# JVBSouza/descriptools

Hardware: AMD Instinct MI355X
Metric: Mcells/s full descriptor chain (higher is better)
Workload: dtype f32; 1 GPU; 16384x16384 synthetic tilted-integer-fBm DEM per GPU, full chain (d8, flowacc, river mask, flowhand/HAND with fused GFI + ln(hl/H), fused slope+TI+MTI, downslope), device-resident; global_dem=16384x16384, river_threshold_cells=524288

## Files before the change

descriptools_amd/csrc/dt_capi.hip:

```cpp
#include <cmath>
#include <stdarg.h>
#include <stdlib.h>

#include <sys/mman.h>
#include <atomic>
#include <chrono>
#include <mutex>
#include <system_error>
#include <thread>
#include <utility>
#include <vector>

#include "dt_common.h"
#include "dt_kernels.h"

static thread_local char g_err[512] = "";
void dt_set_error(const char *fmt, ...) {
  va_list ap;
  va_start(ap, fmt);
  vsnprintf(g_err, sizeof(g_err), fmt, ap);
  va_end(ap);
}
extern "C" const char *dt_last_error(void) { return g_err; }
extern "C" const char *dt_version(void) { return "descriptools_hip 0.1 (gfx950)"; }
// ... 1135 lines not shown
}

static int dev_flowacc_river_flowhand_local(dt_ctx *c, const uint8_t *fdr, const float *dem, const uint8_t *nod4,
                                           int64_t H, int64_t W, int64_t threshold, int32_t *acc32, int8_t *river,
                                           const DtTwiEpilogue *twi = nullptr) {
  DT_CTX(c);
  DT_TRY(dt_check_hw(H, W));
  DT_REQUIRE((fdr && acc32 && river) || H * W == 0, "NULL raster");
  DT_REQUIRE(!twi || H * W == 0 || dt_twi_epilogue_ok(dt_full_window(H, W), acc32, river, twi),
             "this raster does not take the TI / MTI epilogue (dt_slope_from_d8_ok): use dt_dev_slope_twi");
  size_t need = dt_flowacc_tiled_scratch(H, W), need2 = dt_flowhand_tiled_scratch(H, W);
  DT_TRY(dt_scratch_reset(c, need + need2 + 512));
  void *scr = dt_scratch_take(c, need), *scr2 = dt_scratch_take(c, need2);
  DT_REQUIRE(scr && scr2, "scratch reservation failed");
  DtWin w = dt_full_window(H, W);
  DT_TRY(dt_launch_fa_local(c->stream, w, fdr, scr, need, acc32, 0));
  DT_TRY(dt_launch_fa_finish_fh_local(c->stream, w, fdr, dem, scr, scr2, need2, nullptr, threshold, acc32, 0, river,
                                      c->status, nod4, dt_nodata4_ld(W), twi));
  DT_HIP(hipGetLastError());
  c->scratch_owner = 2;
  c->owner_h = H;
  c->owner_w = W;
  c->owner_ptr = (char *)scr2;
  c->owner_ptr2 = nullptr;
  return DT_OK;
}
extern "C" int dt_dev_flowacc_river_flowhand_local(dt_ctx *c, const uint8_t *fdr, const float *dem, int64_t H, int64_t W,
                                                   int64_t threshold, int32_t *acc32, int8_t *river) {
  return dev_flowacc_river_flowhand_local(c, fdr, dem, nullptr, H, W, threshold, acc32, river);
}
extern "C" int dt_dev_flowacc_river_flowhand_local_m(dt_ctx *c, const uint8_t *fdr, const float *dem,
                                                     const uint8_t *nodata4, int64_t H, int64_t W, int64_t threshold,
                                                     int32_t *acc32, int8_t *river) {
// ... 1117 lines not shown
```

descriptools_amd/csrc/dt_common.h:

```cpp
#pragma once
#include <hip/hip_runtime.h>
#include <stdint.h>
#include <stdio.h>
#include <string.h>

#include "../../include/descriptools_hip.h"

#define DT_NODATA (-100.0f)

void dt_set_error(const char *fmt, ...);

#define DT_HIP(call)                                                                   \
  do {                                                                                 \
    hipError_t e__ = (call);                                                           \
    if (e__ != hipSuccess) {                                                           \
      dt_set_error("%s failed: %s (%s:%d)", #call, hipGetErrorString(e__), __FILE__,   \
                   __LINE__);                                                          \
      return e__ == hipErrorOutOfMemory ? DT_ENOMEM : DT_EHIP;                         \
    }                                                                                  \
  } while (0)

#define DT_REQUIRE(cond, msg)                      \
  do {                                             \
    if (!(cond)) {                                 \
      dt_set_error("invalid argument: %s", msg);   \
      return DT_EINVAL;                            \
    }                                              \
  } while (0)

#define DT_TRY(expr)          \
  do {                        \
    int rc__ = (expr);        \
    if (rc__ != DT_OK) return rc__; \
  } while (0)

enum { DT_DBG_TWI_FLAG_ALL = 0, DT_DBG_TWI_PLAIN = 1, DT_DBG_TWI_WX = 2, DT_DBG_TWI_MAP = 3, DT_DBG_DS_MARGIN = 4, DT_DBG_NO_FUSED_FA_FH = 5, DT_DBG_HY_FILL_SWEEPS = 6, DT_DBG_HY_FLAT_SWEEPS = 7, DT_DBG_HY_COLOUR_MIN = 8 , DT_DBG_FA_SCATTER = 9 , DT_DBG_RC_SLOTS = 10 , DT_DBG_COUNT = 11 };
#define DT_TWI_WX_DEFAULT 1
int dt_debug_get(int key);

struct dt_ctx {
  int device;
  hipStream_t stream;
  bool own_stream;
  char *scratch;
  size_t scratch_bytes;
  size_t scratch_used;
  int scratch_owner;
  int64_t owner_h, owner_w;
  char *owner_ptr;
  char *owner_ptr2;
  char *scratch2;
// ... 36 lines not shown
__host__ __device__ __forceinline__ bool dt_readable(const DtWin &w, int y, int x) {
  int gy = w.gy0 + y, gx = w.gx0 + x;
  return gy >= 0 && gy < w.Hg && gx >= 0 && gx < w.Wg && y >= -w.halo && y < w.H + w.halo && x >= -w.halo &&
         x < w.W + w.halo;
}
__host__ __device__ __forceinline__ bool dt_has_code(const DtWin &w, int y, int x) {
  if (!dt_readable(w, y, x)) return false;
  const int gy = w.gy0 + y, gx = w.gx0 + x;
  return (y > -w.halo || gy == 0) && (y < w.H + w.halo - 1 || gy == w.Hg - 1) && (x > -w.halo || gx == 0) &&
         (x < w.W + w.halo - 1 || gx == w.Wg - 1);
}
__host__ __device__ __forceinline__ bool dt_in_global(const DtWin &w, int y, int x) {
  int gy = w.gy0 + y, gx = w.gx0 + x;
  return gy >= 0 && gy < w.Hg && gx >= 0 && gx < w.Wg;
}
__host__ __device__ __forceinline__ long long dt_perim_count(int H, int W) {
  if (H <= 0 || W <= 0) return 0;
  if (H == 1) return W;
  if (W == 1) return H;
  return 2ll * W + 2ll * (H - 2);
}
__host__ __device__ __forceinline__ long long dt_perim_index(int H, int W, int y, int x) {
  if (H == 1) return x;
  if (W == 1) return y;
  if (y == 0) return x;
  if (y == H - 1) return (long long)W + x;
  if (x == 0) return 2ll * W + (y - 1);
  if (x == W - 1) return 2ll * W + (H - 2) + (y - 1);
  return -1;
}
// ... 9 lines not shown
```

descriptools_amd/csrc/dt_fa3fh1_kernel.inc:

```
#if FA3_TWI
__global__ __launch_bounds__(256, 6) void k_fa3fh1_twi(const uint8_t *__restrict__ fdr, const float *__restrict__ dem,
#else
template <int ND>
__global__ __launch_bounds__(256, 6) void k_fa3fh1(const uint8_t *__restrict__ fdr, const float *__restrict__ dem,
#endif
                                                  const uint8_t *__restrict__ nod4, int ldm, DtWin w, int tiles_x,
                                                  const unsigned long long *__restrict__ rec,
                                                  const unsigned long long *__restrict__ state,
                                                  const unsigned long long *__restrict__ ext,
                                                  const uint16_t *__restrict__ loc16, int32_t *__restrict__ acc32,
                                                  int32_t river_thr, int8_t *__restrict__ river,
                                                  int *__restrict__ status, uint32_t nnodes,
                                                  unsigned long long *__restrict__ nodes,
                                                  unsigned long long *__restrict__ cache,
#if FA3_TWI
                                                  uint8_t *__restrict__ cache_wide, TwiOut tw) {
  constexpr int ND = 2;
#else
                                                  uint8_t *__restrict__ cache_wide) {
#endif
#define P3(c) ((uint32_t)(c) + (((uint32_t)(c) >> 6) << 2))
#define NT3 (TH * (TW + 4))
  __shared__ __attribute__((aligned(16))) unsigned char smem[NT3 * 6];
  __shared__ unsigned long long s_in;
  __shared__ int s_ovf;
  uint32_t *s_delta = reinterpret_cast<uint32_t *>(smem);
  uint16_t *s_nxt = reinterpret_cast<uint16_t *>(smem + NT3 * 4);
  const int tile = dt_tile_of_block((int)blockIdx.x, (int)gridDim.x);
  const int ty = tile / tiles_x, tx = tile - ty * tiles_x;
  const int y0 = ty * TH, x0 = tx * TW;
  const uint4 v_fdr = dt_tile_fetch16(fdr, w, y0, x0);
  uint32_t c2[8] = {0u, 0u, 0u, 0u, 0u, 0u, 0u, 0u};
  if (rec) fa_nbr_codes(fdr, w, y0, x0, threadIdx.x, c2);
  unsigned long long e = 0ull;
// ... 29 lines not shown
    const bool interior = dt_tile_interior(w, y0, x0);
    const int pbase = ly * (TW + 4) + lxb;
#pragma unroll
    for (int q = 0; q < 4; q++) {
      uint32_t nn[4];
#pragma unroll
      for (int k = 0; k < 4; k++) {
        const uint32_t code = (cv[q] >> (8 * k)) & 0xFFu;
        const int lx = lxb + 4 * q + k;
        const uint32_t n = interior ? dt_tile_next_interior(code, ly, lx) : dt_tile_next(code, ly, lx, y0, x0, w);
        nn[k] = n < NT ? P3(n) : n;
      }
      *reinterpret_cast<uint2 *>(&s_nxt[pbase + 4 * q]) = make_uint2(nn[0] | (nn[1] << 16), nn[2] | (nn[3] << 16));
      *reinterpret_cast<uint4 *>(&s_delta[pbase + 4 * q]) = make_uint4(0, 0, 0, 0);
    }
  }
  if (rec) e = fa_inflow(fa_gather(c2, y0, x0, threadIdx.x, tiles_x, rec, state), e);
  if (threadIdx.x == 0) s_ovf = 0;
  if (__syncthreads_or(!(e & FA_CYCLE) && FA_VALUE(e) >= (1ull << 22))) {
    if (threadIdx.x == 0) s_in = 0ull;
    __syncthreads();
    if (e != 0ull && !(e & FA_CYCLE)) atomicAdd(&s_in, FA_VALUE(e));
    __syncthreads();
    if (threadIdx.x == 0 && s_in >= (1ull << 31) - (unsigned long long)NT && status) atomicOr(status, DT_STATUS_ACC_OVERFLOW);
  }
  if (e != 0ull) {
    int ly, lx;
    dt_cell_of_slot(threadIdx.x, ly, lx);
    uint32_t c = P3(ly * TW + lx);
    if (e & FA_CYCLE) {
// ... 57 lines not shown
        tw.tile_mark[stile] = (uint8_t)1;
      }
    }
#endif
  }
  __syncthreads();
#undef P3
#undef NT3
  uint32_t *s_w = reinterpret_cast<uint32_t *>(smem);
  uint8_t *s_fdr = smem + NT * 4;
  uint8_t *s_kind = smem + NT * 5;
  uint32_t *s_lut = reinterpret_cast<uint32_t *>(smem + NT * 6);
  s_lut[threadIdx.x] = fh_lut_entry(threadIdx.x);
  dt_tile_put16(s_fdr, v_fdr);
  __syncthreads();
  fh_tile1n_body(s_fdr, s_w, s_kind, &s_ovf, s_lut, riv4, w, tile, tiles_x, y0, x0, nnodes, nodes, cache, cache_wide);
}
```

descriptools_amd/csrc/dt_kernels.h:

```cpp
#pragma once
#include "dt_common.h"

int dt_launch_synth_dem(hipStream_t s, uint32_t seed, int O, int64_t Hg, int64_t y0, int64_t x0,
                        int64_t h, int64_t w, int nodata_pct, float *out);
int dt_launch_stencil(hipStream_t s, const DtWin &w, const float *dem, double px, float *slope,
                      uint8_t *fdr, float *slope_rad, const void *acc, int acc64, double n_top, float *ti,
                      float *mti, void *aux = nullptr, uint8_t *nod4 = nullptr, int ldm = 0);
static inline int dt_nodata4_ld(int64_t W) { return (int)((((W + 3) / 4) + 7) & ~(int64_t)7); }
static inline size_t dt_nodata4_bytes(int64_t H, int64_t W) { return (size_t)((H + 3) / 4) * (size_t)dt_nodata4_ld(W) * 2; }
size_t dt_stencil_aux_bytes(int64_t H, int64_t W);
int dt_launch_d8_slope(hipStream_t s, const DtWin &w, const float *dem, double px, uint8_t *fdr, float *slope,
                       void *aux, uint8_t *nod4, int ldm, void *smarks);
int dt_launch_slope_twi_fix(hipStream_t s, const DtWin &w, const float *dem, double px, float *slope,
                            const int32_t *acc, double n_top, float *ti, float *mti, void *smarks);
int dt_launch_flowacc(hipStream_t s, const uint8_t *fdr, const float *dem, int64_t H, int64_t W,
                      unsigned long long *state, int32_t *acc32);
int dt_launch_river_mask(hipStream_t s, const int32_t *acc32, int64_t n, int64_t thr, int8_t *river);
int dt_launch_flowhand(hipStream_t s, const float *dem, const uint8_t *fdr, const int8_t *river,
                       const int32_t *acc32, int64_t H, int64_t W, double px,
                       unsigned long long *state, float *fdist, int32_t *idx32, float *hand,
                       int32_t *a_river);
int dt_launch_twi(hipStream_t s, const int32_t *acc32, const float *srad, int64_t n, double px,
                  double n_top, float *ti, float *mti);
int dt_launch_twi_i64(hipStream_t s, const int64_t *fac, const float *srad, int64_t n, double px,
// ... 48 lines not shown
                             const int64_t *idx64, const void *fac, const void *a_river, int acc64, int64_t n_remote,
                             const uint8_t *res_ok, const int64_t *rem_gidx, const double *rem_zr64, void *table,
                             double expo, double b, double size, double *hand, float *gfi, float *lnhlh);
int dt_launch_ds_walk_f64(hipStream_t s, const DtWin &w, const double *dem, const uint8_t *fdr, double px, double dz,
                          int64_t n, void *rec, float *out);
int dt_launch_ds_walk_seed_f64(hipStream_t s, const DtWin &w, const double *dem, int64_t n, const int32_t *ys,
                               const int32_t *xs, void *rec);
int dt_launch_confusion(hipStream_t s, const double *desc, const int8_t *flood, int64_t n,
                        double nodata, const double *th_host, int nth, int under,
                        unsigned long long *counts4);
int dt_launch_i32_to_i64(hipStream_t s, const int32_t *a, int64_t n, int64_t *b);
int dt_launch_i64_to_i32(hipStream_t s, const int64_t *a, int64_t n, int32_t *b);

size_t dt_flowacc_tiled_scratch(int64_t H, int64_t W);
int dt_launch_fa_local(hipStream_t s, const DtWin &w, const uint8_t *fdr, void *scratch, size_t scratch_bytes,
                       int32_t *acc32, int rank_level);
int dt_launch_fa_summary(hipStream_t s, const DtWin &w, void *scratch, int64_t *A, int32_t *xr, uint8_t *code);
int dt_launch_fa_finish(hipStream_t s, const DtWin &w, const uint8_t *fdr, const float *dem, void *scratch,
                        const unsigned long long *ext_perim, int64_t river_thr, void *acc, int acc64,
                        int8_t *river, int *status = nullptr);
size_t dt_flowacc_weighted_scratch(int64_t H, int64_t W);
int dt_launch_flowacc_weighted(hipStream_t s, const DtWin &w, const uint8_t *fdr, const float *dem, const double *wt,
                               int frac_bits, void *scratch, size_t scratch_bytes, double *acc, int *status);
size_t dt_flowhand_tiled_scratch(int64_t H, int64_t W);
struct DtTwiEpilogue {
  const float *slope;
  float *ti, *mti;
  double px, n_top;
  void *marks;
};
int dt_launch_fa_finish_fh_local(hipStream_t s, const DtWin &w, const uint8_t *fdr, const float *dem, void *fa_scratch,
                                 void *fh_scratch, size_t fh_bytes, const unsigned long long *ext_perim,
                                 int64_t river_thr, void *acc, int acc64, int8_t *river, int *status,
                                 const uint8_t *nod4 = nullptr, int ldm = 0, const DtTwiEpilogue *twi = nullptr);
bool dt_twi_epilogue_ok(const DtWin &w, const void *acc, const int8_t *river, const DtTwiEpilogue *twi);
int dt_launch_fh_local(hipStream_t s, const DtWin &w, const uint8_t *fdr, const int8_t *river, void *scratch,
                       size_t scratch_bytes);
int dt_launch_fh_summary(hipStream_t s, const DtWin &w, void *scratch, const float *dem, const void *acc, int acc64,
                         uint8_t *kind, int32_t *ref, int32_t *nc, int32_t *nd, float *zr, long long *ar);
int dt_launch_fh_finish(hipStream_t s, const DtWin &w, const float *dem, const uint8_t *fdr,
                        const int8_t *river, const void *acc, int acc64, double px, void *scratch,
                        const uint8_t *res_ok, const int32_t *res_nc, const int32_t *res_nd,
                        const long long *rem_gidx, const float *rem_zr, const long long *rem_ar, float *fdist,
                        int32_t *idx32, long long *idx64, float *hand, void *a_river, float *gfi = nullptr,
                        float *lnhlh = nullptr, double n_gfi = 0.0, double b_gfi = 1.0, double size = 1.0);
int dt_launch_gfi_both(hipStream_t s, const float *hand, const void *a_river, const void *fac, int acc64,
                       int64_t n, double expo, double b, double size, float *gfi, float *lnhlh);
int dt_launch_unique_extremes(hipStream_t s, const float *x, int64_t n, uint32_t *work4, float *out3);
int dt_launch_minmax_scale(hipStream_t s, const float *x, int64_t n, float mn, float mx, float nodata,
// ... 69 lines not shown
```

descriptools_amd/csrc/dt_tiles.hip:

```cpp
#include "dt_common.h"
#include "dt_kernels.h"
#include "dt_math.h"

#define TW 64
#define TH 64
#define NT (TW * TH)
#define PS (2 * TW + 2 * (TH - 2))
#define CPT (NT / 256)

#define NX_SINK 0xFFFFu
#define NX_EXIT 0xFFFEu
#define NX_REXIT 0xFFFDu
#define X_NONE 0xFFFFu

__device__ __forceinline__ int dt_slot_of(int ly, int lx) {
  if (ly == 0) return lx;
  if (ly == TH - 1) return TW + lx;
  if (lx == 0) return 2 * TW + (ly - 1);
  if (lx == TW - 1) return 2 * TW + (TH - 2) + (ly - 1);
  return -1;
}
__device__ __forceinline__ void dt_cell_of_slot(int s, int &ly, int &lx) {
  if (s < TW) { ly = 0; lx = s; }
  else if (s < 2 * TW) { ly = TH - 1; lx = s - TW; }
// ... 270 lines not shown
  }
#pragma unroll
  for (int j = 0; j < CPT / 2; j++) {
    int c2 = threadIdx.x + 256 * j;
    uint32_t cy = *reinterpret_cast<const uint16_t *>(&s_cyc[2 * c2]);
    uint32_t a = (cy & 0xFFu) ? 0xFFFFu : (va[j] - 1u) & 0xFFFFu;
    uint32_t b = (cy & 0xFF00u) ? 0xFFFFu : (vb[j] - 1u) & 0xFFFFu;
    *reinterpret_cast<uint32_t *>(loc16 + (size_t)tile * NT + 2 * c2) = a | (b << 16);
  }
}

__global__ __launch_bounds__(256) void k_fa_reduce(const unsigned long long *__restrict__ rec, int64_t nnodes,
                                                  const uint32_t *__restrict__ entry_of,
                                                  const uint32_t *__restrict__ parent,
                                                  unsigned long long *__restrict__ state,
                                                  unsigned long long *__restrict__ ext) {
  const int64_t n = (int64_t)blockIdx.x * 256 + threadIdx.x;
  if (ext) {
    if (n >= nnodes) return;
    unsigned long long r = rec[n];
    if (REC_CODE(r) == 0) return;
    if (state[n] != 0ull) return;
    unsigned long long A = REC_W(r);
    uint32_t e = entry_of[n], p = parent[n];
    for (int64_t it = 0; it < nnodes; it++) {
      if (e == FA_NONE) break;
      atomicAdd(&ext[e], A);
      if (p == FA_NONE) break;
      unsigned long long rp = rec[p];
      uint32_t ep = entry_of[p], pp = parent[p];
      unsigned long long old = atomicAdd(&state[p], A - (1ull << FA2_SH));
      if ((old >> FA2_SH) != 1ull) break;
// ... 354 lines not shown
  return f;
}
struct FaIn {
  const unsigned long long *rec, *state, *ext;
};
static FaIn fa_inputs(const FaScratch &f, const unsigned long long *ext_perim) {
  if (dt_debug_get(DT_DBG_FA_SCATTER)) return FaIn{nullptr, nullptr, f.ext};
  return FaIn{f.rec, f.state, ext_perim ? f.ext : nullptr};
}
size_t dt_flowacc_tiled_scratch(int64_t H, int64_t W) {
  int64_t ntiles = ((W + TW - 1) / TW) * ((H + TH - 1) / TH);
  size_t nn = (size_t)ntiles * PS;
  return dt_align256(nn * 8) * 3 + dt_align256(nn * 4) * 3 + 256 + dt_align256((size_t)ntiles * NT * 2);
}

int dt_launch_fa_local(hipStream_t s, const DtWin &w, const uint8_t *fdr, void *scratch, size_t scratch_bytes,
                       int32_t *acc32, int rank_level) {
  if (w.H == 0 || w.W == 0) return DT_OK;
  DT_REQUIRE(scratch_bytes >= dt_flowacc_tiled_scratch(w.H, w.W), "scratch too small");
  FaScratch f = fa_layout(w, scratch);
  DT_REQUIRE(f.nnodes < 0x7FFFFFF0ll, "raster too large for one device tile");
  dim3 gt((unsigned)f.ntiles), b(256), gn((unsigned)((f.nnodes + 255) / 256));
  (void)acc32;
  const bool scatter = dt_debug_get(DT_DBG_FA_SCATTER) != 0;
  hipLaunchKernelGGL(k_fa_tile1, gt, b, 0, s, fdr, w, f.tiles_x, f.rec, f.loc16, f.state,
                     (rank_level || scatter) ? f.ext : nullptr, f.entry_of, f.parent);
  hipLaunchKernelGGL(k_fa_reduce, gn, b, 0, s, f.rec, f.nnodes, f.entry_of, f.parent, f.state, scatter ? f.ext : nullptr);
  if (rank_level) {
    hipLaunchKernelGGL(k_fa_nxt_init, gn, b, 0, s, f.rec, f.nnodes, f.entry_of, f.state, f.nxt);
  }
  return DT_OK;
}

int dt_launch_fa_summary(hipStream_t s, const DtWin &w, void *scratch, int64_t *A, int32_t *xr,
                         uint8_t *code) {
  int64_t P = dt_perim_count(w.H, w.W);
  if (P == 0) return DT_OK;
  FaScratch f = fa_layout(w, scratch);
  hipLaunchKernelGGL(k_fa_rank_summary, dim3((unsigned)((P + 255) / 256)), dim3(256), 0, s, w, f.tiles_x,
                     f.rec, f.state, f.nxt, f.nnodes, P, A, xr, code);
  return DT_OK;
}
// ... 498 lines not shown
  return (ptr & 0x7FFFu) | ((uint32_t)((s >> 16) & 0xFFu) << 15) | ((uint32_t)(s & 0xFFu) << 23);
}
__device__ __forceinline__ unsigned long long fh_cache_unpack(uint32_t v) {
  return fht_pack(v & 0x7FFFu, (v >> 15) & 0xFFu, ((v >> 23) & 0xFFu) | FHT_DONE);
}
__device__ __forceinline__ unsigned long long fh_cache_get(const unsigned long long *__restrict__ cache, bool wide,
                                                            int tile, int c) {
  if (wide) return cache[(size_t)tile * NT + c];
  return fh_cache_unpack(reinterpret_cast<const uint32_t *>(cache + (size_t)tile * NT)[c]);
}

__global__ __launch_bounds__(256) void k_fh_tile1(const uint8_t *__restrict__ fdr,
                                                 const int8_t *__restrict__ river, DtWin w, int tiles_x,
                                                 uint32_t nnodes, unsigned long long *__restrict__ nodes,
                                                 unsigned long long *__restrict__ cache,
                                                 uint8_t *__restrict__ cache_wide, int only_marked, int ntiles) {
  __shared__ __attribute__((aligned(16))) uint8_t s_fdr[NT];
  __shared__ uint8_t s_halo[2 * (TW + 2) + 2 * TH];
  __shared__ __attribute__((aligned(16))) unsigned long long s_st[NT];
  for (int tile = (int)blockIdx.x; tile < ntiles; tile += (int)gridDim.x) {
  if (only_marked && cache_wide[tile] != 2) continue;
  const int ty = tile / tiles_x, tx = tile - ty * tiles_x;
  const int y0 = ty * TH, x0 = tx * TW;
  FhTile T{s_fdr, s_halo, s_st};
  fht_solve_tile(T, fdr, river, w, y0, x0);
  if (threadIdx.x < PS) {
    int ly, lx;
    dt_cell_of_slot(threadIdx.x, ly, lx);
    unsigned long long s = s_st[ly * TW + lx];
    uint32_t ptr = (uint32_t)(s >> 32), nd = (uint32_t)((s >> 16) & 0xFFFFu);
    uint32_t ncf = (uint32_t)(s & 0xFFFFu), nc = ncf & 0x7FFFu;
    uint32_t kind = (ptr >> 12) & 7u, f = ptr & 0xFFFu;
    int fy = (int)f / TW, fx = (int)f % TW;
    unsigned long long o = fht_pack(FHT_DEAD, 0, FHT_DONE);
// ... 35 lines not shown
#define FN_DONE 0x40000u
#define FN_LOW 0x7FFFFu
#define FN_OVF 0x20100u
#define FN_PTR_SH 19
__device__ __forceinline__ uint32_t fh_lut_entry(uint32_t code) {
  if (!dt_d8_valid(code)) return 0u;
  int dy, dx;
  dt_d8_delta(code, dy, dx);
  return ((uint32_t)(dy * TW + dx) << FN_PTR_SH) + ((dy != 0 && dx != 0) ? (1u << 9) : 1u);
}
__device__ __forceinline__ void fh_tile1n_body(uint8_t *s_fdr, uint32_t *s_w, uint8_t *s_kind, int *s_ovf_p,
                                               const uint32_t *s_lut, const uint32_t (&riv4)[NT / 4 / 256],
                                               const DtWin &w, int tile, int tiles_x, int y0, int x0, uint32_t nnodes,
                                               unsigned long long *__restrict__ nodes,
                                               unsigned long long *__restrict__ cache,
                                               uint8_t *__restrict__ cache_wide) {
#define s_ovf (*s_ovf_p)
  const bool interior = dt_tile_interior(w, y0, x0);
  const uint32_t lx0 = (4u * threadIdx.x) & 63u;
#pragma unroll
  for (int u = 0; u < NT / 4 / 256; u++) {
    const int c0 = 4 * (threadIdx.x + 256 * u);
    const uint32_t codes = *reinterpret_cast<const uint32_t *>(&s_fdr[c0]);
    uint32_t wd[4], kinds = 0;
#pragma unroll
    for (int k = 0; k < 4; k++) {
      const int c = c0 + k;
      const uint32_t code = (codes >> (8 * k)) & 0xFFu, cw = (uint32_t)c << FN_PTR_SH;
      const bool is_river = ((riv4[u] >> (8 * k)) & 0xFFu) == 1u;
      uint32_t word = cw | FN_DONE, kind = K_DEAD;
      if (interior) {
// ... 53 lines not shown
      }
      if (!dy) {
        v.y = s_w[v.y >> FN_PTR_SH] + (v.y & FN_CNT);
        if (!(v.y & (FN_DONE | FN_OVF))) v.y = s_w[v.y >> FN_PTR_SH] + (v.y & FN_CNT);
        ovf |= v.y & FN_OVF;
      }
      own[j] = v;
      s_w2[c2] = v;
      changed |= ((v.x & v.y & FN_DONE) == 0u) ? 1 : 0;
    }
    if (ovf) s_ovf = 1;
    if (!__syncthreads_or(changed)) break;
    if (s_ovf) break;
  }
  if (s_ovf) {
    if (threadIdx.x == 0) cache_wide[tile] = 2;
    return;
  }
  auto narrow = [&](uint32_t v, uint32_t c) -> uint32_t {
    uint32_t f = v >> FN_PTR_SH, kind = s_kind[f];
    if (!(v & FN_DONE)) { f = c; kind = K_DEAD; v = 0; }
    return f | (kind << 12) | (((v >> 9) & 0xFFu) << 15) | ((v & 0xFFu) << 23);
  };
#pragma unroll
  for (int j = 0; j < CPT / 2; j++) {
    const int c2 = threadIdx.x + 256 * j;
    s_w2[c2] = make_uint2(narrow(own[j].x, 2u * (uint32_t)c2), narrow(own[j].y, 2u * (uint32_t)c2 + 1u));
  }
  if (threadIdx.x == 0) cache_wide[tile] = 0;
  __syncthreads();
  uint32_t *c32 = reinterpret_cast<uint32_t *>(cache + (size_t)tile * NT);
#pragma unroll
  for (int u = 0; u < NT / 4 / 256; u++) {
    int c = 4 * (threadIdx.x + 256 * u);
    *reinterpret_cast<uint4 *>(c32 + c) = *reinterpret_cast<const uint4 *>(&s_w[c]);
  }
  if (threadIdx.x < PS) {
    int ly, lx;
    dt_cell_of_slot(threadIdx.x, ly, lx);
    unsigned long long sw = fh_cache_unpack(s_w[ly * TW + lx]);
    uint32_t ptr = (uint32_t)(sw >> 32), nd = (uint32_t)((sw >> 16) & 0xFFFFu), nc = (uint32_t)sw & 0x7FFFu;
    uint32_t kind = (ptr >> 12) & 7u, f = ptr & 0xFFFu;
    int fy = (int)f / TW, fx = (int)f % TW;
    unsigned long long o = fht_pack(FHT_DEAD, 0, FHT_DONE);
    if (kind == K_RIVER) {
      o = fht_pack((uint32_t)((y0 + fy) * w.W + x0 + fx), nd, nc | FHT_DONE);
    } else if (kind == K_EXIT || kind == K_REXIT) {
      int dy, dx;
      dt_d8_delta(s_fdr[f], dy, dx);
      bool diag = dy != 0 && dx != 0;
      uint32_t node = kind == K_EXIT ? dt_node_of(y0 + fy + dy, x0 + fx + dx, tiles_x)
                                     : nnodes + (uint32_t)dt_perim_index(w.H, w.W, y0 + fy, x0 + fx);
      o = fht_pack(node, nd + (diag ? 1u : 0u), nc + (diag ? 0u : 1u));
    }
    nodes[(size_t)tile * PS + threadIdx.x] = o;
  }
#undef s_ovf
}

__global__ __launch_bounds__(256, 6) void k_fh_tile1n(const uint8_t *__restrict__ fdr,
// ... 7 lines not shown
  __shared__ uint32_t s_lut[256];
  __shared__ int s_ovf;
  const int tile = dt_tile_of_block((int)blockIdx.x, (int)gridDim.x);
  const int ty = tile / tiles_x, tx = tile - ty * tiles_x;
  const int y0 = ty * TH, x0 = tx * TW;
  const uint4 v_fdr = dt_tile_fetch16(fdr, w, y0, x0);
  const uint4 v_riv = dt_tile_fetch16(reinterpret_cast<const uint8_t *>(river), w, y0, x0);
  dt_tile_put16(s_fdr, v_fdr);
  dt_tile_put16(s_kind, v_riv);
  s_lut[threadIdx.x] = fh_lut_entry(threadIdx.x);
  if (threadIdx.x == 0) s_ovf = 0;
  __syncthreads();
  uint32_t riv4[NT / 4 / 256];
#pragma unroll
  for (int u = 0; u < NT / 4 / 256; u++) riv4[u] = *reinterpret_cast<const uint32_t *>(&s_kind[4 * (threadIdx.x + 256 * u)]);
  fh_tile1n_body(s_fdr, s_w, s_kind, &s_ovf, s_lut, riv4, w, tile, tiles_x, y0, x0, nnodes, nodes, cache, cache_wide);
}


struct TwiOut {
  const float *slope;
  float *ti, *mti;
  double n_top, lnpx2;
  uint8_t *tile_mark;
  uint32_t *lane_mask;
  int stiles_x;
};
typedef float fa_v4f __attribute__((ext_vector_type(4)));
#define FA3_TWI 0
#include "dt_fa3fh1_kernel.inc"
#undef FA3_TWI
// ... 364 lines not shown
  f.tiles_x = (w.W + TW - 1) / TW;
  f.ntiles = (int64_t)f.tiles_x * ((w.H + TH - 1) / TH);
  f.nnodes = f.ntiles * PS;
  f.P = dt_perim_count(w.H, w.W);
  f.nodes = (unsigned long long *)scratch;
  f.cache = (unsigned long long *)((char *)scratch + dt_align256(((size_t)f.nnodes + (size_t)f.P) * 8));
  f.cache_wide = (uint8_t *)f.cache + dt_align256((size_t)f.ntiles * NT * 8) + 256;
  return f;
}
size_t dt_flowhand_tiled_scratch(int64_t H, int64_t W) {
  int64_t ntiles = ((W + TW - 1) / TW) * ((H + TH - 1) / TH);
  return dt_align256(((size_t)ntiles * PS + (size_t)dt_perim_count((int)H, (int)W)) * 8) +
         dt_align256((size_t)ntiles * NT * 8) + 256 + dt_align256((size_t)ntiles);
}

static int fh_local_tail(hipStream_t s, const DtWin &w, const uint8_t *fdr, const int8_t *river, const FhScratch &f) {
  dim3 gt((unsigned)f.ntiles), b(256), gn((unsigned)((f.nnodes + f.P + 255) / 256));
  hipLaunchKernelGGL(k_fh_tile1, dim3(gt.x < 2048u ? gt.x : 2048u), b, 0, s, fdr, river, w, f.tiles_x,
                     (uint32_t)f.nnodes, f.nodes, f.cache, f.cache_wide, 1, (int)f.ntiles);
  hipLaunchKernelGGL(k_fh_ghost_init, dim3((unsigned)((f.P + 255) / 256)), b, 0, s, f.nodes, (uint32_t)f.nnodes, f.P);
  int *flags = (int *)((char *)f.cache + dt_align256((size_t)f.ntiles * NT * 8));
  DT_HIP(hipMemsetAsync(flags, 0, 64, s));
  dim3 gj(gn.x < 4096u ? gn.x : 4096u);
  for (int r = 0; r < 8; r++)
    hipLaunchKernelGGL(k_fh_node_jump, gj, b, 0, s, f.nodes, f.nnodes + f.P, flags, r, 3);
  return DT_OK;
}

int dt_launch_fh_local(hipStream_t s, const DtWin &w, const uint8_t *fdr, const int8_t *river, void *scratch,
                       size_t scratch_bytes) {
  if (w.H == 0 || w.W == 0) return DT_OK;
  DT_REQUIRE(scratch_bytes >= dt_flowhand_tiled_scratch(w.H, w.W), "scratch too small");
  FhScratch f = fh_layout(w, scratch);
  DT_REQUIRE(f.nnodes + f.P < 0x7FFFFFF0ll, "raster too large for one device tile");
  hipLaunchKernelGGL(k_fh_tile1n, dim3((unsigned)f.ntiles), dim3(256), 0, s, fdr, river, w, f.tiles_x,
                     (uint32_t)f.nnodes, f.nodes, f.cache, f.cache_wide);
  return fh_local_tail(s, w, fdr, river, f);
}

bool dt_twi_epilogue_ok(const DtWin &w, const void *acc, const int8_t *river, const DtTwiEpilogue *twi) {
  return dt_debug_get(DT_DBG_NO_FUSED_FA_FH) == 0 && w.W % TW == 0 && (w.ld & 3) == 0 && w.halo == 0 && w.gx0 == 0 &&
         w.gy0 == 0 && w.ld == w.W && ((uintptr_t)acc & 15) == 0 && ((uintptr_t)river & 3) == 0 && twi->marks &&
         twi->slope && twi->ti && twi->mti &&
         (((uintptr_t)twi->slope | (uintptr_t)twi->ti | (uintptr_t)twi->mti | (uintptr_t)twi->marks) & 15) == 0;
}

int dt_launch_fa_finish_fh_local(hipStream_t s, const DtWin &w, const uint8_t *fdr, const float *dem, void *fa_scratch,
                                 void *fh_scratch, size_t fh_bytes, const unsigned long long *ext_perim,
                                 int64_t river_thr, void *acc, int acc64, int8_t *river, int *status,
                                 const uint8_t *nod4, int ldm, const DtTwiEpilogue *twi) {
  if (w.H == 0 || w.W == 0) return DT_OK;
  DT_REQUIRE(fh_bytes >= dt_flowhand_tiled_scratch(w.H, w.W), "scratch too small");
  DT_REQUIRE(river != nullptr, "HAND needs the river mask");
  FaScratch f = fa_layout(w, fa_scratch);
  FhScratch h = fh_layout(w, fh_scratch);
  DT_REQUIRE(h.nnodes + h.P < 0x7FFFFFF0ll, "raster too large for one device tile");
  dim3 gt((unsigned)f.ntiles), b(256), gn((unsigned)((f.nnodes + 255) / 256));
  if (ext_perim) {
    int64_t P = dt_perim_count(w.H, w.W);
    hipLaunchKernelGGL(k_fa_propagate, dim3((unsigned)((P + 255) / 256)), b, 0, s, w, f.tiles_x, f.nnodes, f.nxt,
                       ext_perim, P, f.ext);
  }
  if (dt_debug_get(DT_DBG_FA_SCATTER)) hipLaunchKernelGGL(k_fa_poison, gn, b, 0, s, f.rec, f.nnodes, f.entry_of, f.state, f.ext);
  const bool fused = !acc64 && dt_debug_get(DT_DBG_NO_FUSED_FA_FH) == 0 && w.W % TW == 0 && (w.ld & 3) == 0 &&
                     (((uintptr_t)acc | (uintptr_t)dem) & 15) == 0 && ((uintptr_t)river & 3) == 0;
  if (fused) {
    const FaIn in = fa_inputs(f, ext_perim);
    int32_t thr = river_thr > 2147483647ll ? 2147483647 : (river_thr < -2147483647ll ? -2147483647 : (int32_t)river_thr);
    const bool use_mask = nod4 != nullptr && w.halo == 0 && w.gx0 == 0 && w.gy0 == 0;
    if (twi) {
      DT_REQUIRE(dt_twi_epilogue_ok(w, acc, river, twi) && use_mask && !ext_perim,
                 "the TI / MTI epilogue takes a single raster with its nodata mask (dt_twi_epilogue_ok)");
      const int64_t stx = (w.W + 255) / 256, sntiles = stx * ((w.H + 15) / 16);
      TwiOut tw{twi->slope, twi->ti, twi->mti, twi->n_top, log(twi->px * twi->px), (uint8_t *)twi->marks,
                (uint32_t *)((char *)twi->marks + dt_align256((size_t)sntiles)), (int)stx};
      hipLaunchKernelGGL(k_fa3fh1_twi, gt, b, 0, s, fdr, dem, nod4, ldm, w, f.tiles_x, in.rec, in.state, in.ext, f.loc16,
                         (int32_t *)acc, thr, river, status, (uint32_t)h.nnodes, h.nodes, h.cache, h.cache_wide, tw);
    } else if (use_mask)
      hipLaunchKernelGGL(k_fa3fh1<2>, gt, b, 0, s, fdr, dem, nod4, ldm, w, f.tiles_x, in.rec, in.state, in.ext, f.loc16, (int32_t *)acc, thr,
                         river, status, (uint32_t)h.nnodes, h.nodes, h.cache, h.cache_wide);
    else if (dem)
      hipLaunchKernelGGL(k_fa3fh1<1>, gt, b, 0, s, fdr, dem, nod4, ldm, w, f.tiles_x, in.rec, in.state, in.ext, f.loc16, (int32_t *)acc, thr,
                         river, status, (uint32_t)h.nnodes, h.nodes, h.cache, h.cache_wide);
    else
      hipLaunchKernelGGL(k_fa3fh1<0>, gt, b, 0, s, fdr, dem, nod4, ldm, w, f.tiles_x, in.rec, in.state, in.ext, f.loc16, (int32_t *)acc, thr,
                         river, status, (uint32_t)h.nnodes, h.nodes, h.cache, h.cache_wide);
  } else {
    DT_REQUIRE(!twi, "the TI / MTI epilogue needs the fused form of the tile passes (dt_twi_epilogue_ok)");
    if (acc64) {
      fa_launch_tile3<long long>(s, gt, w, fdr, dem, f, ext_perim, (long long *)acc, (long long)river_thr, river, status);
    } else {
      int32_t thr = river_thr > 2147483647ll ? 2147483647 : (river_thr < -2147483647ll ? -2147483647 : (int32_t)river_thr);
      fa_launch_tile3<int32_t>(s, gt, w, fdr, dem, f, ext_perim, (int32_t *)acc, thr, river, status);
    }
    hipLaunchKernelGGL(k_fh_tile1n, gt, b, 0, s, fdr, river, w, h.tiles_x, (uint32_t)h.nnodes, h.nodes, h.cache,
                       h.cache_wide);
  }
  return fh_local_tail(s, w, fdr, river, h);
}

int dt_launch_fh_summary(hipStream_t s, const DtWin &w, void *scratch, const float *dem, const void *acc, int acc64,
                         uint8_t *kind, int32_t *ref, int32_t *nc, int32_t *nd, float *zr, long long *ar) {
  FhScratch f = fh_layout(w, scratch);
  if (f.P == 0) return DT_OK;
  dim3 g((unsigned)((f.P + 255) / 256)), b(256);
  if (acc64)
    hipLaunchKernelGGL(k_fh_rank_summary<long long>, g, b, 0, s, w, f.tiles_x, (uint32_t)f.nnodes, f.nodes, dem,
                       (const long long *)acc, f.P, kind, ref, nc, nd, zr, ar);
  else
    hipLaunchKernelGGL(k_fh_rank_summary<int32_t>, g, b, 0, s, w, f.tiles_x, (uint32_t)f.nnodes, f.nodes, dem,
                       (const int32_t *)acc, f.P, kind, ref, nc, nd, zr, ar);
  return DT_OK;
}
// ... 298 lines not shown
```

Before: 35960 Mcells/s.

## Skip dead flowhand nodes, early-exit overflow tile pass, drop ghost init and memset

In the fused flowacc+flowhand tile kernel, each node gets a liveness flag (it has inflow, a back-pointing neighbour, or lies on a non-whole window border), and dead nodes get a DEAD record instead of a resolved one. Overflowing tiles count themselves in a control word, and the later overflow-tile pass exits at once when that count is zero. For whole-raster windows the ghost-node init is skipped and the jump passes cover only real nodes. The control-word memset is folded into the flowacc reduce kernel. This trims launches and node-jump work, and it relies on the liveness test being exact for correctness.

```diff
diff --git a/descriptools_amd/csrc/dt_capi.hip b/descriptools_amd/csrc/dt_capi.hip
--- a/descriptools_amd/csrc/dt_capi.hip
+++ b/descriptools_amd/csrc/dt_capi.hip
@@ -1173,9 +1173,9 @@
   void *scr = dt_scratch_take(c, need), *scr2 = dt_scratch_take(c, need2);
   DT_REQUIRE(scr && scr2, "scratch reservation failed");
   DtWin w = dt_full_window(H, W);
-  DT_TRY(dt_launch_fa_local(c->stream, w, fdr, scr, need, acc32, 0));
+  DT_TRY(dt_launch_fa_local(c->stream, w, fdr, scr, need, acc32, 0, scr2));
   DT_TRY(dt_launch_fa_finish_fh_local(c->stream, w, fdr, dem, scr, scr2, need2, nullptr, threshold, acc32, 0, river,
-                                      c->status, nod4, dt_nodata4_ld(W), twi));
+                                      c->status, nod4, dt_nodata4_ld(W), twi, true));
   DT_HIP(hipGetLastError());
   c->scratch_owner = 2;
   c->owner_h = H;
diff --git a/descriptools_amd/csrc/dt_common.h b/descriptools_amd/csrc/dt_common.h
--- a/descriptools_amd/csrc/dt_common.h
+++ b/descriptools_amd/csrc/dt_common.h
@@ -34,7 +34,7 @@
     if (rc__ != DT_OK) return rc__; \
   } while (0)
 
-enum { DT_DBG_TWI_FLAG_ALL = 0, DT_DBG_TWI_PLAIN = 1, DT_DBG_TWI_WX = 2, DT_DBG_TWI_MAP = 3, DT_DBG_DS_MARGIN = 4, DT_DBG_NO_FUSED_FA_FH = 5, DT_DBG_HY_FILL_SWEEPS = 6, DT_DBG_HY_FLAT_SWEEPS = 7, DT_DBG_HY_COLOUR_MIN = 8 , DT_DBG_FA_SCATTER = 9 , DT_DBG_RC_SLOTS = 10 , DT_DBG_COUNT = 11 };
+enum { DT_DBG_TWI_FLAG_ALL = 0, DT_DBG_TWI_PLAIN = 1, DT_DBG_TWI_WX = 2, DT_DBG_TWI_MAP = 3, DT_DBG_DS_MARGIN = 4, DT_DBG_NO_FUSED_FA_FH = 5, DT_DBG_HY_FILL_SWEEPS = 6, DT_DBG_HY_FLAT_SWEEPS = 7, DT_DBG_HY_COLOUR_MIN = 8 , DT_DBG_FA_SCATTER = 9 , DT_DBG_RC_SLOTS = 10 , DT_DBG_FH_ALL_NODES = 11 , DT_DBG_COUNT = 12 };
 #define DT_TWI_WX_DEFAULT 1
 int dt_debug_get(int key);
 
@@ -101,6 +101,9 @@
   int gy = w.gy0 + y, gx = w.gx0 + x;
   return gy >= 0 && gy < w.Hg && gx >= 0 && gx < w.Wg;
 }
+__host__ __device__ __forceinline__ bool dt_win_is_whole(const DtWin &w) {
+  return w.gy0 == 0 && w.gx0 == 0 && w.Hg == w.H && w.Wg == w.W;
+}
 __host__ __device__ __forceinline__ long long dt_perim_count(int H, int W) {
   if (H <= 0 || W <= 0) return 0;
   if (H == 1) return W;
diff --git a/descriptools_amd/csrc/dt_fa3fh1_kernel.inc b/descriptools_amd/csrc/dt_fa3fh1_kernel.inc
--- a/descriptools_amd/csrc/dt_fa3fh1_kernel.inc
+++ b/descriptools_amd/csrc/dt_fa3fh1_kernel.inc
@@ -13,11 +13,12 @@
                                                   int *__restrict__ status, uint32_t nnodes,
                                                   unsigned long long *__restrict__ nodes,
                                                   unsigned long long *__restrict__ cache,
+                                                  uint8_t *__restrict__ cache_wide, int *__restrict__ given_up,
 #if FA3_TWI
-                                                  uint8_t *__restrict__ cache_wide, TwiOut tw) {
+                                                  int all_nodes, TwiOut tw) {
   constexpr int ND = 2;
 #else
-                                                  uint8_t *__restrict__ cache_wide) {
+                                                  int all_nodes) {
 #endif
 #define P3(c) ((uint32_t)(c) + (((uint32_t)(c) >> 6) << 2))
 #define NT3 (TH * (TW + 4))
@@ -77,6 +78,14 @@
       *reinterpret_cast<uint2 *>(&s_nxt[pbase + 4 * q]) = make_uint2(nn[0] | (nn[1] << 16), nn[2] | (nn[3] << 16));
       *reinterpret_cast<uint4 *>(&s_delta[pbase + 4 * q]) = make_uint4(0, 0, 0, 0);
     }
+  }
+  bool live = rec == nullptr || all_nodes != 0 || e != 0ull;
+#pragma unroll
+  for (int q = 0; q < 8; q++) live = live || c2[q] == fa_back(q);
+  if (!dt_win_is_whole(w) && threadIdx.x < PS) {
+    int ly, lx;
+    dt_cell_of_slot(threadIdx.x, ly, lx);
+    live = live || y0 + ly == 0 || y0 + ly == w.H - 1 || x0 + lx == 0 || x0 + lx == w.W - 1;
   }
   if (rec) e = fa_inflow(fa_gather(c2, y0, x0, threadIdx.x, tiles_x, rec, state), e);
   if (threadIdx.x == 0) s_ovf = 0;
@@ -164,5 +173,6 @@
   s_lut[threadIdx.x] = fh_lut_entry(threadIdx.x);
   dt_tile_put16(s_fdr, v_fdr);
   __syncthreads();
-  fh_tile1n_body(s_fdr, s_w, s_kind, &s_ovf, s_lut, riv4, w, tile, tiles_x, y0, x0, nnodes, nodes, cache, cache_wide);
+  fh_tile1n_body(s_fdr, s_w, s_kind, &s_ovf, s_lut, riv4, w, tile, tiles_x, y0, x0, nnodes, nodes, cache, cache_wide, live,
+                 given_up);
 }
diff --git a/descriptools_amd/csrc/dt_kernels.h b/descriptools_amd/csrc/dt_kernels.h
--- a/descriptools_amd/csrc/dt_kernels.h
+++ b/descriptools_amd/csrc/dt_kernels.h
@@ -86,7 +86,7 @@
 
 size_t dt_flowacc_tiled_scratch(int64_t H, int64_t W);
 int dt_launch_fa_local(hipStream_t s, const DtWin &w, const uint8_t *fdr, void *scratch, size_t scratch_bytes,
-                       int32_t *acc32, int rank_level);
+                       int32_t *acc32, int rank_level, void *fh_scratch = nullptr);
 int dt_launch_fa_summary(hipStream_t s, const DtWin &w, void *scratch, int64_t *A, int32_t *xr, uint8_t *code);
 int dt_launch_fa_finish(hipStream_t s, const DtWin &w, const uint8_t *fdr, const float *dem, void *scratch,
                         const unsigned long long *ext_perim, int64_t river_thr, void *acc, int acc64,
@@ -104,7 +104,8 @@
 int dt_launch_fa_finish_fh_local(hipStream_t s, const DtWin &w, const uint8_t *fdr, const float *dem, void *fa_scratch,
                                  void *fh_scratch, size_t fh_bytes, const unsigned long long *ext_perim,
                                  int64_t river_thr, void *acc, int acc64, int8_t *river, int *status,
-                                 const uint8_t *nod4 = nullptr, int ldm = 0, const DtTwiEpilogue *twi = nullptr);
+                                 const uint8_t *nod4 = nullptr, int ldm = 0, const DtTwiEpilogue *twi = nullptr,
+                                 bool fh_ctl_zeroed = false);
 bool dt_twi_epilogue_ok(const DtWin &w, const void *acc, const int8_t *river, const DtTwiEpilogue *twi);
 int dt_launch_fh_local(hipStream_t s, const DtWin &w, const uint8_t *fdr, const int8_t *river, void *scratch,
                        size_t scratch_bytes);
diff --git a/descriptools_amd/csrc/dt_tiles.hip b/descriptools_amd/csrc/dt_tiles.hip
--- a/descriptools_amd/csrc/dt_tiles.hip
+++ b/descriptools_amd/csrc/dt_tiles.hip
@@ -308,8 +308,9 @@
                                                   const uint32_t *__restrict__ entry_of,
                                                   const uint32_t *__restrict__ parent,
                                                   unsigned long long *__restrict__ state,
-                                                  unsigned long long *__restrict__ ext) {
+                                                  unsigned long long *__restrict__ ext, int *__restrict__ zero16) {
   const int64_t n = (int64_t)blockIdx.x * 256 + threadIdx.x;
+  if (zero16 && n < 16) zero16[n] = 0;
   if (ext) {
     if (n >= nnodes) return;
     unsigned long long r = rec[n];
@@ -694,8 +695,9 @@
   return dt_align256(nn * 8) * 3 + dt_align256(nn * 4) * 3 + 256 + dt_align256((size_t)ntiles * NT * 2);
 }
 
+static int *fh_ctl_of(const DtWin &w, void *fh_scratch);
 int dt_launch_fa_local(hipStream_t s, const DtWin &w, const uint8_t *fdr, void *scratch, size_t scratch_bytes,
-                       int32_t *acc32, int rank_level) {
+                       int32_t *acc32, int rank_level, void *fh_scratch) {
   if (w.H == 0 || w.W == 0) return DT_OK;
   DT_REQUIRE(scratch_bytes >= dt_flowacc_tiled_scratch(w.H, w.W), "scratch too small");
   FaScratch f = fa_layout(w, scratch);
@@ -705,7 +707,8 @@
   const bool scatter = dt_debug_get(DT_DBG_FA_SCATTER) != 0;
   hipLaunchKernelGGL(k_fa_tile1, gt, b, 0, s, fdr, w, f.tiles_x, f.rec, f.loc16, f.state,
                      (rank_level || scatter) ? f.ext : nullptr, f.entry_of, f.parent);
-  hipLaunchKernelGGL(k_fa_reduce, gn, b, 0, s, f.rec, f.nnodes, f.entry_of, f.parent, f.state, scatter ? f.ext : nullptr);
+  hipLaunchKernelGGL(k_fa_reduce, gn, b, 0, s, f.rec, f.nnodes, f.entry_of, f.parent, f.state, scatter ? f.ext : nullptr,
+                     fh_scratch ? fh_ctl_of(w, fh_scratch) : (int *)nullptr);
   if (rank_level) {
     hipLaunchKernelGGL(k_fa_nxt_init, gn, b, 0, s, f.rec, f.nnodes, f.entry_of, f.state, f.nxt);
   }
@@ -1234,10 +1237,12 @@
                                                  const int8_t *__restrict__ river, DtWin w, int tiles_x,
                                                  uint32_t nnodes, unsigned long long *__restrict__ nodes,
                                                  unsigned long long *__restrict__ cache,
-                                                 uint8_t *__restrict__ cache_wide, int only_marked, int ntiles) {
+                                                 uint8_t *__restrict__ cache_wide, int only_marked, int ntiles,
+                                                 const int *__restrict__ given_up) {
   __shared__ __attribute__((aligned(16))) uint8_t s_fdr[NT];
   __shared__ uint8_t s_halo[2 * (TW + 2) + 2 * TH];
   __shared__ __attribute__((aligned(16))) unsigned long long s_st[NT];
+  if (given_up && *given_up == 0) return;
   for (int tile = (int)blockIdx.x; tile < ntiles; tile += (int)gridDim.x) {
   if (only_marked && cache_wide[tile] != 2) continue;
   const int ty = tile / tiles_x, tx = tile - ty * tiles_x;
@@ -1303,7 +1308,8 @@
                                                const DtWin &w, int tile, int tiles_x, int y0, int x0, uint32_t nnodes,
                                                unsigned long long *__restrict__ nodes,
                                                unsigned long long *__restrict__ cache,
-                                               uint8_t *__restrict__ cache_wide) {
+                                               uint8_t *__restrict__ cache_wide, bool live,
+                                               int *__restrict__ given_up) {
 #define s_ovf (*s_ovf_p)
   const bool interior = dt_tile_interior(w, y0, x0);
   const uint32_t lx0 = (4u * threadIdx.x) & 63u;
@@ -1387,7 +1393,10 @@
     if (s_ovf) break;
   }
   if (s_ovf) {
-    if (threadIdx.x == 0) cache_wide[tile] = 2;
+    if (threadIdx.x == 0) {
+      cache_wide[tile] = 2;
+      if (given_up) atomicAdd(given_up, 1);
+    }
     return;
   }
   auto narrow = [&](uint32_t v, uint32_t c) -> uint32_t {
@@ -1416,7 +1425,8 @@
     uint32_t kind = (ptr >> 12) & 7u, f = ptr & 0xFFFu;
     int fy = (int)f / TW, fx = (int)f % TW;
     unsigned long long o = fht_pack(FHT_DEAD, 0, FHT_DONE);
-    if (kind == K_RIVER) {
+    if (!live) {
+    } else if (kind == K_RIVER) {
       o = fht_pack((uint32_t)((y0 + fy) * w.W + x0 + fx), nd, nc | FHT_DONE);
     } else if (kind == K_EXIT || kind == K_REXIT) {
       int dy, dx;
@@ -1454,7 +1464,8 @@
   uint32_t riv4[NT / 4 / 256];
 #pragma unroll
   for (int u = 0; u < NT / 4 / 256; u++) riv4[u] = *reinterpret_cast<const uint32_t *>(&s_kind[4 * (threadIdx.x + 256 * u)]);
-  fh_tile1n_body(s_fdr, s_w, s_kind, &s_ovf, s_lut, riv4, w, tile, tiles_x, y0, x0, nnodes, nodes, cache, cache_wide);
+  fh_tile1n_body(s_fdr, s_w, s_kind, &s_ovf, s_lut, riv4, w, tile, tiles_x, y0, x0, nnodes, nodes, cache, cache_wide, true,
+                 nullptr);
 }
 
 
@@ -1849,16 +1860,26 @@
          dt_align256((size_t)ntiles * NT * 8) + 256 + dt_align256((size_t)ntiles);
 }
 
-static int fh_local_tail(hipStream_t s, const DtWin &w, const uint8_t *fdr, const int8_t *river, const FhScratch &f) {
-  dim3 gt((unsigned)f.ntiles), b(256), gn((unsigned)((f.nnodes + f.P + 255) / 256));
+#define FH_GIVEN_UP 8
+#define FH_CTL_BYTES 64
+static int *fh_ctl(const FhScratch &f) { return (int *)((char *)f.cache + dt_align256((size_t)f.ntiles * NT * 8)); }
+static int *fh_ctl_of(const DtWin &w, void *fh_scratch) { return fh_ctl(fh_layout(w, fh_scratch)); }
+static_assert(FH_CTL_BYTES == 16 * sizeof(int), "k_fa_reduce clears 16 ints");
+
+static int fh_local_tail(hipStream_t s, const DtWin &w, const uint8_t *fdr, const int8_t *river, const FhScratch &f,
+                         bool counted) {
+  const bool ghosts = !dt_win_is_whole(w);
+  const int64_t nn = f.nnodes + (ghosts ? f.P : 0);
+  dim3 gt((unsigned)f.ntiles), b(256), gn((unsigned)((nn + 255) / 256));
+  int *ctl = fh_ctl(f);
   hipLaunchKernelGGL(k_fh_tile1, dim3(gt.x < 2048u ? gt.x : 2048u), b, 0, s, fdr, river, w, f.tiles_x,
-                     (uint32_t)f.nnodes, f.nodes, f.cache, f.cache_wide, 1, (int)f.ntiles);
-  hipLaunchKernelGGL(k_fh_ghost_init, dim3((unsigned)((f.P + 255) / 256)), b, 0, s, f.nodes, (uint32_t)f.nnodes, f.P);
-  int *flags = (int *)((char *)f.cache + dt_align256((size_t)f.ntiles * NT * 8));
-  DT_HIP(hipMemsetAsync(flags, 0, 64, s));
+                     (uint32_t)f.nnodes, f.nodes, f.cache, f.cache_wide, 1, (int)f.ntiles,
+                     counted ? ctl + FH_GIVEN_UP : (const int *)nullptr);
+  if (ghosts)
+    hipLaunchKernelGGL(k_fh_ghost_init, dim3((unsigned)((f.P + 255) / 256)), b, 0, s, f.nodes, (uint32_t)f.nnodes, f.P);
   dim3 gj(gn.x < 4096u ? gn.x : 4096u);
   for (int r = 0; r < 8; r++)
-    hipLaunchKernelGGL(k_fh_node_jump, gj, b, 0, s, f.nodes, f.nnodes + f.P, flags, r, 3);
+    hipLaunchKernelGGL(k_fh_node_jump, gj, b, 0, s, f.nodes, nn, ctl, r, 3);
   return DT_OK;
 }
 
@@ -1868,9 +1889,10 @@
   DT_REQUIRE(scratch_bytes >= dt_flowhand_tiled_scratch(w.H, w.W), "scratch too small");
   FhScratch f = fh_layout(w, scratch);
   DT_REQUIRE(f.nnodes + f.P < 0x7FFFFFF0ll, "raster too large for one device tile");
+  DT_HIP(hipMemsetAsync(fh_ctl(f), 0, FH_CTL_BYTES, s));
   hipLaunchKernelGGL(k_fh_tile1n, dim3((unsigned)f.ntiles), dim3(256), 0, s, fdr, river, w, f.tiles_x,
                      (uint32_t)f.nnodes, f.nodes, f.cache, f.cache_wide);
-  return fh_local_tail(s, w, fdr, river, f);
+  return fh_local_tail(s, w, fdr, river, f, false);
 }
 
 bool dt_twi_epilogue_ok(const DtWin &w, const void *acc, const int8_t *river, const DtTwiEpilogue *twi) {
@@ -1883,7 +1905,7 @@
 int dt_launch_fa_finish_fh_local(hipStream_t s, const DtWin &w, const uint8_t *fdr, const float *dem, void *fa_scratch,
                                  void *fh_scratch, size_t fh_bytes, const unsigned long long *ext_perim,
                                  int64_t river_thr, void *acc, int acc64, int8_t *river, int *status,
-                                 const uint8_t *nod4, int ldm, const DtTwiEpilogue *twi) {
+                                 const uint8_t *nod4, int ldm, const DtTwiEpilogue *twi, bool fh_ctl_zeroed) {
   if (w.H == 0 || w.W == 0) return DT_OK;
   DT_REQUIRE(fh_bytes >= dt_flowhand_tiled_scratch(w.H, w.W), "scratch too small");
   DT_REQUIRE(river != nullptr, "HAND needs the river mask");
@@ -1899,6 +1921,9 @@
   if (dt_debug_get(DT_DBG_FA_SCATTER)) hipLaunchKernelGGL(k_fa_poison, gn, b, 0, s, f.rec, f.nnodes, f.entry_of, f.state, f.ext);
   const bool fused = !acc64 && dt_debug_get(DT_DBG_NO_FUSED_FA_FH) == 0 && w.W % TW == 0 && (w.ld & 3) == 0 &&
                      (((uintptr_t)acc | (uintptr_t)dem) & 15) == 0 && ((uintptr_t)river & 3) == 0;
+  int *ctl = fh_ctl(h);
+  if (!fh_ctl_zeroed) DT_HIP(hipMemsetAsync(ctl, 0, FH_CTL_BYTES, s));
+  const int all_nodes = dt_debug_get(DT_DBG_FH_ALL_NODES) != 0;
   if (fused) {
     const FaIn in = fa_inputs(f, ext_perim);
     int32_t thr = river_thr > 2147483647ll ? 2147483647 : (river_thr < -2147483647ll ? -2147483647 : (int32_t)river_thr);
@@ -1910,16 +1935,17 @@
       TwiOut tw{twi->slope, twi->ti, twi->mti, twi->n_top, log(twi->px * twi->px), (uint8_t *)twi->marks,
                 (uint32_t *)((char *)twi->marks + dt_align256((size_t)sntiles)), (int)stx};
       hipLaunchKernelGGL(k_fa3fh1_twi, gt, b, 0, s, fdr, dem, nod4, ldm, w, f.tiles_x, in.rec, in.state, in.ext, f.loc16,
-                         (int32_t *)acc, thr, river, status, (uint32_t)h.nnodes, h.nodes, h.cache, h.cache_wide, tw);
+                         (int32_t *)acc, thr, river, status, (uint32_t)h.nnodes, h.nodes, h.cache, h.cache_wide, ctl + FH_GIVEN_UP,
+                         all_nodes, tw);
     } else if (use_mask)
       hipLaunchKernelGGL(k_fa3fh1<2>, gt, b, 0, s, fdr, dem, nod4, ldm, w, f.tiles_x, in.rec, in.state, in.ext, f.loc16, (int32_t *)acc, thr,
-                         river, status, (uint32_t)h.nnodes, h.nodes, h.cache, h.cache_wide);
+                         river, status, (uint32_t)h.nnodes, h.nodes, h.cache, h.cache_wide, ctl + FH_GIVEN_UP, all_nodes);
     else if (dem)
       hipLaunchKernelGGL(k_fa3fh1<1>, gt, b, 0, s, fdr, dem, nod4, ldm, w, f.tiles_x, in.rec, in.state, in.ext, f.loc16, (int32_t *)acc, thr,
-                         river, status, (uint32_t)h.nnodes, h.nodes, h.cache, h.cache_wide);
+                         river, status, (uint32_t)h.nnodes, h.nodes, h.cache, h.cache_wide, ctl + FH_GIVEN_UP, all_nodes);
     else
       hipLaunchKernelGGL(k_fa3fh1<0>, gt, b, 0, s, fdr, dem, nod4, ldm, w, f.tiles_x, in.rec, in.state, in.ext, f.loc16, (int32_t *)acc, thr,
-                         river, status, (uint32_t)h.nnodes, h.nodes, h.cache, h.cache_wide);
+                         river, status, (uint32_t)h.nnodes, h.nodes, h.cache, h.cache_wide, ctl + FH_GIVEN_UP, all_nodes);
   } else {
     DT_REQUIRE(!twi, "the TI / MTI epilogue needs the fused form of the tile passes (dt_twi_epilogue_ok)");
     if (acc64) {
@@ -1931,7 +1957,7 @@
     hipLaunchKernelGGL(k_fh_tile1n, gt, b, 0, s, fdr, river, w, h.tiles_x, (uint32_t)h.nnodes, h.nodes, h.cache,
                        h.cache_wide);
   }
-  return fh_local_tail(s, w, fdr, river, h);
+  return fh_local_tail(s, w, fdr, river, h, fused);
 }
 
 int dt_launch_fh_summary(hipStream_t s, const DtWin &w, void *scratch, const float *dem, const void *acc, int acc64,
```

Measured after the change: 36270 Mcells/s (median of 6 runs). Within noise of the previous version (+0.9%).
